# barathanaslan/whisper-ipa

Measured on AMD Instinct MI355X. Metric: audio-seconds/sec transcribed (whisper-small, 30s clips), higher is better.
Workload: dtype bf16

## Files before the change

include/wipa.h:

```cpp
#ifndef WIPA_H
#define WIPA_H
#include <stddef.h>
#include <stdint.h>
#ifdef __cplusplus
extern "C" {
#endif

typedef void* wipa_stream_t;

enum { WIPA_F32 = 0, WIPA_BF16 = 1, WIPA_FP8_E4M3 = 2  };
enum { WIPA_OK = 0, WIPA_ERR_ARG = -1, WIPA_ERR_HIP = -2, WIPA_ERR_STATE = -3 };

#define WIPA_N_SAMPLES 480000
#define WIPA_N_FRAMES 3000
#define WIPA_N_FFT 400
#define WIPA_HOP 160
#define WIPA_HEAD_DIM 64

int wipa_version(void);
const char* wipa_last_error(void);

int wipa_stream_create(wipa_stream_t* out);
int wipa_stream_create_cu_limited(int n_cus, wipa_stream_t* out);
int wipa_stream_destroy(wipa_stream_t s);
// ... 137 lines not shown
    const float* slabs;
    const float* bias_o;
    const float* ln_w;
    const float* ln_b;
    const void* wq;
    const float* bq;
    const void* kv;
    void* out;
    int64_t slab_stride;
    int32_t n_slabs, B, d, H, Tk, dtype;
    float eps, qk_scale;
    int32_t cross_splits;
} wipa_cross_block_desc;
int wipa_decode_cross_block(const wipa_cross_block_desc* d, wipa_stream_t s);

int wipa_cross_absorbed_splits(int want, int Tk);
int wipa_cross_absorbed_resident_groups_for(int B, int d, int Tk, int n_splits, int64_t budget_bytes);
int wipa_cross_absorbed_resident_groups(int B, int d, int Tk, int n_splits);
size_t wipa_cross_absorbed_scratch_bytes(int B, int d, int Tk);
int wipa_cross_absorbed_init(int d);
int wipa_cross_absorbed_attention(const void* q, int64_t q_row_stride, const void* wkT, const void* xa, const void* wv, const float* bv,
                                  void* out, int64_t out_row_stride, void* scratch, size_t scratch_bytes, int B, int H, int d, int Tk,
                                  float k_scale, int n_splits, wipa_stream_t s);
int wipa_decode_cross_absorbed_block(const wipa_cross_block_desc* c, const void* wkT, const void* wv, const float* bv, void* scratch,
                                     size_t scratch_bytes, wipa_stream_t s);
int wipa_decode_cross_absorbed_block_out(const wipa_cross_block_desc* c, const void* wkT, const void* wv, const float* bv, const void* wo,
                                         const float* bo, float* slabs_out, int64_t slab_stride, void* scratch, size_t scratch_bytes,
                                         wipa_stream_t s);
int wipa_cross_absorbed_stream(const void* xa, void* scratch, size_t scratch_bytes, int B, int H, int d, int Tk, int n_splits,
                               wipa_stream_t s);

int wipa_greedy_step(const float* logits, int64_t ldl, int B, int V, const float* mask_first,
                     const float* mask_always, int32_t* tokens, int64_t ld_tok, const int32_t* pos_dev, int n_init,
                     int eot, float* sum_logprobs, int32_t* not_done, wipa_stream_t s);
int wipa_add_i32(int32_t* p, int32_t v, wipa_stream_t s);
int wipa_greedy_step_embed(const float* logits, int64_t ldl, int B, int V, const float* mask_first, const float* mask_always,
                           int32_t* tokens, int64_t ld_tok, int32_t* pos_dev, int64_t* posd_dev, int32_t* done_counter, int n_init,
                           int eot, float* sum_logprobs, int32_t* not_done, const void* tok_emb, int emb_dtype,
                           const float* emb_scale, const float* pos_emb, int n_ctx, float* x, const float* ln_w, const float* ln_b,
                           void* y, int y_dtype, int D, float eps, wipa_stream_t s);
#define WIPA_GREEDY_PARTS 2048
int wipa_logits_greedy_supported(int B, int V, int d, int dtype);
size_t wipa_logits_greedy_partials_bytes(int B);
int wipa_logits_greedy(const void* x, int64_t ldx, const void* w, int64_t ldw, float* logits, int64_t ldl, int B, int V, int d,
                       const float* mask_first, const float* mask_always, const int32_t* pos_dev, int n_init, float* partials,
                       size_t partials_bytes, wipa_stream_t s);
// ... 196 lines not shown
```

whisper_ipa_amd/_lib.py:

```python
from __future__ import annotations

import ctypes as C
import os
import threading

_HERE = os.path.dirname(os.path.abspath(__file__))
LIB_PATH = os.path.join(_HERE, "libwipa.so")

WIPA_F32, WIPA_BF16, WIPA_FP8_E4M3 = 0, 1, 2
GREEDY_PARTS = 2048
RESAMPLE_TILE = 512
SCORE_MAX_LEN = 1024
ENC_GLOBAL, ENC_PER_LAYER = 7, 14
DEC_GLOBAL, DEC_PER_LAYER, DEC_FP8_PER_LAYER = 4, 20, 6
GEMM_DISPATCH = ("tile128", "tile256", "tile384", "tile384n", "tile256p", "skinny", "skinny_fp8", "skinny_ln", "kmajor", "split_k",
                 "tile_fp8", "tile_fp8_384")
ENC_FP8_PER_LAYER = 8
DEC_ABSORBED_PER_LAYER = 1

c_void_p, c_int, c_int64, c_size_t, c_float = C.c_void_p, C.c_int, C.c_int64, C.c_size_t, C.c_float


class GemmDesc(C.Structure):
    _fields_ = [
# ... 88 lines not shown
                               c_float, c_void_p]),
    "wipa_layernorm_fp8": (c_int, [c_void_p, c_int64, c_void_p, c_int64, c_void_p, c_void_p, c_void_p, c_int, c_int, c_float, c_void_p]),
    "wipa_rowquant_fp8": (c_int, [c_void_p, c_int, c_int64, c_void_p, c_int64, c_void_p, c_int, c_int, c_void_p]),
    "wipa_add_slabs_layernorm": (c_int, [c_void_p, c_int64, c_void_p, c_int, c_int64, c_void_p, c_int, c_int64, c_void_p,
                                         c_void_p, c_int, c_int, c_float, c_void_p]),
    "wipa_embed_tokens": (c_int, [c_void_p, c_int64, c_int, c_int, c_int, c_void_p, c_void_p, c_int, c_void_p, c_void_p, c_void_p,
                                  c_int, c_void_p]),
    "wipa_attention": (c_int, [_P(AttnDesc), c_void_p]),
    "wipa_flash_attn_enc_f32": (c_int, [c_void_p, c_int64, c_void_p, c_int64, c_void_p, c_int64, c_void_p, c_int64, c_int, c_int,
                                       c_int, c_int, c_void_p]),
    "wipa_flash_attn_enc_bf16": (c_int, [c_void_p, c_int64, c_void_p, c_int64, c_void_p, c_int64, c_int, c_int, c_int,
                                         c_void_p]),
    "wipa_decode_attn": (c_int, [_P(AttnDesc), c_void_p]),
    "wipa_decode_cross_attn": (c_int, [c_void_p, c_void_p, c_void_p, c_int, c_int, c_int, c_int, c_void_p]),
    "wipa_decode_self_block": (c_int, [_P(SelfBlockDesc), c_void_p]),
    "wipa_decode_cross_block": (c_int, [_P(CrossBlockDesc), c_void_p]),
    "wipa_cross_absorbed_splits": (c_int, [c_int, c_int]),
    "wipa_cross_absorbed_resident_groups_for": (c_int, [c_int, c_int, c_int, c_int, c_int64]),
    "wipa_cross_absorbed_resident_groups": (c_int, [c_int, c_int, c_int, c_int]),
    "wipa_cross_absorbed_scratch_bytes": (c_size_t, [c_int, c_int, c_int]),
    "wipa_cross_absorbed_init": (c_int, [c_int]),
    "wipa_cross_absorbed_attention": (c_int, [c_void_p, c_int64, c_void_p, c_void_p, c_void_p, c_void_p, c_void_p, c_int64, c_void_p, c_size_t,
                                              c_int, c_int, c_int, c_int, c_float, c_int, c_void_p]),
    "wipa_cross_absorbed_stream": (c_int, [c_void_p, c_void_p, c_size_t, c_int, c_int, c_int, c_int, c_int, c_void_p]),
    "wipa_decode_cross_absorbed_block": (c_int, [_P(CrossBlockDesc), c_void_p, c_void_p, c_void_p, c_void_p, c_size_t, c_void_p]),
    "wipa_decode_cross_absorbed_block_out": (c_int, [_P(CrossBlockDesc), c_void_p, c_void_p, c_void_p, c_void_p, c_void_p, c_void_p, c_int64,
                                                     c_void_p, c_size_t, c_void_p]),
    "wipa_greedy_step": (c_int, [c_void_p, c_int64, c_int, c_int, c_void_p, c_void_p, c_void_p, c_int64, c_void_p, c_int,
                                 c_int, c_void_p, c_void_p, c_void_p]),
    "wipa_add_i32": (c_int, [c_void_p, C.c_int32, c_void_p]),
    "wipa_greedy_step_embed": (c_int, [c_void_p, c_int64, c_int, c_int, c_void_p, c_void_p, c_void_p, c_int64, c_void_p, c_void_p, c_void_p,
                                       c_int, c_int, c_void_p, c_void_p, c_void_p, c_int, c_void_p, c_void_p, c_int, c_void_p, c_void_p,
                                       c_void_p, c_void_p, c_int, c_int, c_float, c_void_p]),
    "wipa_timestamp_step": (c_int, [c_void_p, c_int64, c_int, c_int, c_void_p, c_void_p, c_void_p, c_int64, c_void_p, c_int, c_int,
                                    _P(DecodeRules), c_void_p, c_void_p, c_void_p]),
    "wipa_timestamp_step_embed": (c_int, [c_void_p, c_int64, c_int, c_int, c_void_p, c_void_p, c_void_p, c_int64, c_void_p, c_void_p, c_void_p,
                                          c_int, c_int, _P(DecodeRules), c_void_p, c_void_p, c_void_p, c_int, c_void_p, c_void_p, c_int,
                                          c_void_p, c_void_p, c_void_p, c_void_p, c_int, c_int, c_float, c_void_p]),
    "wipa_sample_record_bytes": (c_size_t, [c_int]),
    "wipa_sample_record_fill": (c_int, [c_void_p, c_size_t, C.c_uint64, c_int, c_float, c_void_p, c_int]),
    "wipa_sample_step": (c_int, [c_void_p, c_int64, c_int, c_int, c_void_p, c_void_p, c_void_p, c_int64, c_void_p, c_int, c_int,
                                 _P(DecodeRules), c_void_p, c_void_p, c_void_p, c_void_p]),
    "wipa_sample_step_embed": (c_int, [c_void_p, c_int64, c_int, c_int, c_void_p, c_void_p, c_void_p, c_int64, c_void_p, c_void_p, c_void_p,
                                       c_int, c_int, _P(DecodeRules), c_void_p, c_void_p, c_void_p, c_void_p, c_int, c_void_p, c_void_p, c_int,
                                       c_void_p, c_void_p, c_void_p, c_void_p, c_int, c_int, c_float, c_void_p]),
    "wipa_sample_noise": (c_int, [c_void_p, c_int, c_int, c_int, c_void_p, c_void_p]),
# ... 118 lines not shown
```

whisper_ipa_amd/csrc/cross_absorbed.hip:

```cpp
#include <cstdlib>
#include <mutex>
#include <type_traits>

#include "attn_stream.h"
#include "wipa_common.h"

int wipa_cross_absorbed_loop_variant() {
    const char* e = getenv("WIPA_ABS_LOOP");
    const int v = e ? atoi(e) : 1;
    return (v >= 0 && v <= 3) ? v : 1;
}

namespace {

constexpr int FT = 32;
constexpr long long XA_RESIDENT_MB_SHARED = 16;
constexpr long long XA_RESIDENT_MB_LONE = -1;
typedef __attribute__((address_space(3))) void* lds_ptr_a;
typedef int v2i32 __attribute__((ext_vector_type(2)));

struct AbsParams {
    const __bf16* qp;
    const __bf16* xa;
    float* part_m;
    float* part_l;
    float* part_o;
    int Tk, n_splits, tiles_per_split, H;
    int resident_groups;
};

constexpr int POLICY_DEFAULT = 0, POLICY_NT = 2;

__device__ __forceinline__ int swz(int row) { return (row & 7) << 1; }

template <int D>
struct AbsCfg {
    static constexpr int NW = 4;
    static constexpr int ROWB = D * 2;
    static constexpr int TILE = FT * ROWB;
    static constexpr int SX = NW * 2 * 64 * 4 * (int)sizeof(float);
    static constexpr int NBUF = (3 * TILE + SX <= 160 * 1024) ? 3 : 2;
    static constexpr int SMEM = NBUF * TILE + SX;
};

template <int D>
__global__ __launch_bounds__(512, 1) void cross_absorbed_kernel(AbsParams p) {
    typedef AbsCfg<D> X;
    constexpr int NW = X::NW, ROWB = X::ROWB, TILE = X::TILE, NBUF = X::NBUF;
    constexpr int NDMA = TILE / 1024 / NW;
    constexpr int KS = D / NW / 32;
    constexpr int CT = D / NW / 16;
// ... 242 lines not shown
    return fmaxf(__uint_as_float(r[0]), __uint_as_float(r[1]));
}
__device__ __forceinline__ float sum_xor16(float v) {
    const auto r = __builtin_amdgcn_permlane16_swap(__float_as_uint(v), __float_as_uint(v), false, false);
    return __uint_as_float(r[0]) + __uint_as_float(r[1]);
}
__device__ __forceinline__ float sum_xor32(float v) {
    const auto r = __builtin_amdgcn_permlane32_swap(__float_as_uint(v), __float_as_uint(v), false, false);
    return __uint_as_float(r[0]) + __uint_as_float(r[1]);
}

template <int D, int NW_, bool PIPE>
__global__ __launch_bounds__(64 * NW_, 1) void cross_absorbed_v2_kernel(AbsParams p) {
    typedef AbsCfg2<D, NW_> X;
    constexpr int NWV = X::NWV, GF = X::GF, ROWB = X::ROWB, SLOT = X::SLOT;
    constexpr int NDMA = SLOT / 1024;
    constexpr int KS = D / 32;
    constexpr int CT = D / 16;
    static_assert(SLOT % 1024 == 0 && NDMA <= 32 && CT % 8 == 0 && KS % 4 == 0 && CT / 8 <= 8 && D % 128 == 0, "width");
    extern __shared__ __attribute__((aligned(1024))) char smem[];
    const int tid = threadIdx.x, lane = tid & 63;
    const int wave = __builtin_amdgcn_readfirstlane(tid >> 6);
    const int l15 = lane & 15, g = lane >> 4;
    const int split = blockIdx.x, b = blockIdx.y;
    const int groups_total = (p.Tk + GF - 1) / GF;
    const int gps = 2 * p.tiles_per_split;
    const int g0 = split * gps;
    const int ng = max(0, min(gps, groups_total - g0));
    const int my_n = ng > wave ? (ng - wave + NWV - 1) / NWV : 0;
    const __bf16* xb = p.xa + (int64_t)b * p.Tk * D;
    char* my = smem + wave * (2 * SLOT);

    bf16x8 qf[KS];
    {
        const __bf16* qr = p.qp + ((int64_t)b * 16 + l15) * D + 8 * g;
#pragma unroll
        for (int ks = 0; ks < KS; ++ks) qf[ks] = *reinterpret_cast<const bf16x8*>(qr + 32 * ks);
    }
    const __amdgpu_buffer_rsrc_t rX = __builtin_amdgcn_make_buffer_rsrc((void*)xb, 0, 0x7fffffff, 0x00020000);
    constexpr int G1K = (ROWB % 1024 == 0) ? 1024 : ((ROWB % 512 == 0) ? 512 : 256);
    constexpr int PER = ROWB / G1K, QR = 1024 / G1K;
    static_assert(NDMA % PER == 0 && PER <= 3 && (QR == 1 || QR == 2 || QR == 4), "transfer / row period");
    int dma_a[PER], dma_b[PER];
#pragma unroll
    for (int t = 0; t < PER; ++t) {
        const int off = 1024 * t + 16 * lane;
        const int r = off / ROWB, c = (off - r * ROWB) >> 4;
        dma_a[t] = (c ^ (r << 1)) << 4;
        dma_b[t] = r * ROWB;
    }
    int lane_v = lane;
    auto stage_as = [&](auto policy, int i_local, int slot) {
        constexpr int AUX = decltype(policy)::value;
        const int f0 = (g0 + wave + NWV * i_local) * GF;
        if (f0 + GF <= p.Tk) {
#pragma unroll
            for (int i = 0; i < NDMA; ++i) {
                const int j = i / PER, t = i % PER;
// ... 166 lines not shown
            (void)scores(slot, i, mx);
            mt = fmaxf(mt, mx);
            asm volatile("s_waitcnt lgkmcnt(0)" ::: "memory");
            if (i + 2 < my_n) stage(i + 2, slot);
        }
        m_ref = mt;
        exact = true;
    }
    const float m_run = m_ref;
    asm volatile("s_waitcnt vmcnt(0)" ::: "memory");
    __syncthreads();
    constexpr int RS = X::MROW;
    float* so = reinterpret_cast<float*>(smem);
    float* sm = so + NWV * 16 * RS;
#pragma unroll
    for (int c = 0; c < CT; ++c)
#pragma unroll
        for (int r = 0; r < 4; ++r) so[(wave * 16 + 4 * g + r) * RS + 16 * c + l15] = acc[c][r];
    if (g == 0) {
        sm[wave * 16 + l15] = m_run;
        sm[NWV * 16 + wave * 16 + l15] = l_run;
    }
    __syncthreads();
    const int64_t ps = (int64_t)b * p.n_splits + split;
    float* po = p.part_o + ps * 16 * D;
    for (int hd = 0; hd < p.H; ++hd) {
        float mv[NWV], M = NEG_BIG;
#pragma unroll
        for (int v = 0; v < NWV; ++v) {
            mv[v] = sm[v * 16 + hd];
            M = fmaxf(M, mv[v]);
        }
        float wgt[NWV];
#pragma unroll
        for (int v = 0; v < NWV; ++v) wgt[v] = __expf(mv[v] - M);
        for (int c4 = tid; 4 * c4 < D; c4 += NWV * 64) {
            f32x4 o = {0.f, 0.f, 0.f, 0.f};
#pragma unroll
            for (int v = 0; v < NWV; ++v)
                o += wgt[v] * *reinterpret_cast<const f32x4*>(so + (v * 16 + hd) * RS + 4 * c4);
            *reinterpret_cast<f32x4*>(po + hd * D + 4 * c4) = o;
        }
    }
    if (tid < 16) {
        float M = NEG_BIG, Lsum = 0.f;
#pragma unroll
        for (int v = 0; v < NWV; ++v) M = fmaxf(M, sm[v * 16 + tid]);
#pragma unroll
        for (int v = 0; v < NWV; ++v) Lsum += __expf(sm[v * 16 + tid] - M) * sm[NWV * 16 + v * 16 + tid];
        p.part_m[ps * 16 + tid] = M;
        p.part_l[ps * 16 + tid] = Lsum;
    }
}
#undef WIPA_TR8
#undef WIPA_TR8_ISSUE
#undef WIPA_TR8_NEXT
#undef WIPA_TR8_LAST

template <int D>
__global__ __launch_bounds__(64) void cross_absorb_q_kernel(const __bf16* __restrict__ q, int64_t q_rs, const __bf16* __restrict__ wkT,
                                                            __bf16* __restrict__ qp, int B, int H, float scale) {
    constexpr int CT = D / 4 / 16;
    const int lane = threadIdx.x & 63, wave = blockIdx.z;
    const int l15 = lane & 15, g = lane >> 4;
    const int h = blockIdx.x, b0 = blockIdx.y * 16;
    if (h >= H) {
        for (int e = lane; e < 16 * (D / 4); e += 64) {
            const int bb = b0 + e / (D / 4);
            if (bb < B) qp[((int64_t)bb * 16 + h) * D + wave * (D / 4) + e % (D / 4)] = (__bf16)0.f;
        }
        return;
    }
    const int bq = min(b0 + l15, B - 1);
    bf16x8 qa[2];
#pragma unroll
    for (int ks = 0; ks < 2; ++ks) qa[ks] = *reinterpret_cast<const bf16x8*>(q + (int64_t)bq * q_rs + h * 64 + 32 * ks + 8 * g);
    bf16x8 wb[CT][2];
#pragma unroll
    for (int i = 0; i < CT; ++i)
#pragma unroll
        for (int ks = 0; ks < 2; ++ks)
            wb[i][ks] = *reinterpret_cast<const bf16x8*>(wkT + (int64_t)(wave * (D / 4) + 16 * i + l15) * D + h * 64 + 32 * ks + 8 * g);
#pragma unroll
    for (int i = 0; i < CT; ++i) {
        const int c0 = wave * (D / 4) + 16 * i;
        f32x4 acc = f32x4{0.f, 0.f, 0.f, 0.f};
// ... 6 lines not shown
        }
    }
}

template <int D>
struct MergeCfg {
#ifndef WIPA_MERGE_KQ
#define WIPA_MERGE_KQ 96
#endif
#ifndef WIPA_MERGE_CL
#define WIPA_MERGE_CL 4
#endif
    static constexpr int KQ = (D % 96 == 0) ? WIPA_MERGE_KQ : (D == 512 ? 64 : 128);
    static constexpr int NWM = D / KQ;
    static constexpr int KS = KQ / 32;
    static constexpr int CL = WIPA_MERGE_CL;
};

template <int D, bool OUTP = false, int NS = 4>
__global__ __launch_bounds__(64 * MergeCfg<D>::NWM) void cross_merge_proj_kernel(
    const float* __restrict__ part_m, const float* __restrict__ part_l, const float* __restrict__ part_o, int n_splits,
    const __bf16* __restrict__ wv, const float* __restrict__ bv, __bf16* __restrict__ out, int64_t o_rs, int B,
    const __bf16* __restrict__ wo = nullptr, const float* __restrict__ bo = nullptr, float* __restrict__ slabs_out = nullptr,
    int64_t slab_stride = 0) {
    constexpr int KQ = MergeCfg<D>::KQ, KS = MergeCfg<D>::KS, NWM = MergeCfg<D>::NWM;
    static_assert(KQ % 32 == 0 && NWM * KQ == D, "width");
    constexpr int CL = MergeCfg<D>::CL;
    constexpr int NTO = D / 16;
    constexpr int NTOW = (NTO + NWM - 1) / NWM;
    __shared__ __attribute__((aligned(16))) float red[NWM][CL][64 + 4];
    __shared__ __attribute__((aligned(16))) __bf16 vh[OUTP ? CL : 1][64 + 8];
    const int tid = threadIdx.x, lane = tid & 63, w = tid >> 6;
    const int l15 = lane & 15, g = lane >> 4;
    const int h = blockIdx.x, b0 = blockIdx.y * CL;
    const int bc = min(b0 + (l15 & (CL - 1)), B - 1);
    bf16x8 wq[4][KS];
#pragma unroll
    for (int nt = 0; nt < 4; ++nt)
#pragma unroll
        for (int ks = 0; ks < KS; ++ks)
            wq[nt][ks] = *reinterpret_cast<const bf16x8*>(wv + (int64_t)(h * 64 + 16 * nt + l15) * D + w * KQ + 32 * ks + 8 * g);
    bf16x8 wof[OUTP ? NTOW : 1][2];
    if constexpr (OUTP) {
#pragma unroll
        for (int i = 0; i < NTOW; ++i) {
            const int nt = min(w * NTOW + i, NTO - 1);
#pragma unroll
            for (int ks = 0; ks < 2; ++ks)
// ... 241 lines not shown
                    if (4 * g + r < CG && bb_ < p.B) p.qp[((int64_t)bb_ * 16 + h) * D + 16 * nt + l15] = (__bf16)(acc[r] * p.k_scale);
                }
            }
        }
    }
}

template <int D, bool OUTP, typename... Args>
void launch_merge(int lv, int S, dim3 grid, hipStream_t s, Args... args) {
    constexpr int T = 64 * MergeCfg<D>::NWM;
    const int ns = (lv == 1 || lv == 3) ? S : 4;
    if (ns == 1) hipLaunchKernelGGL((cross_merge_proj_kernel<D, OUTP, 1>), grid, dim3(T), 0, s, args...);
    else if (ns == 2) hipLaunchKernelGGL((cross_merge_proj_kernel<D, OUTP, 2>), grid, dim3(T), 0, s, args...);
    else if (ns == 3) hipLaunchKernelGGL((cross_merge_proj_kernel<D, OUTP, 3>), grid, dim3(T), 0, s, args...);
    else hipLaunchKernelGGL((cross_merge_proj_kernel<D, OUTP, 4>), grid, dim3(T), 0, s, args...);
}

template <int D>
int launch_attn(int lv, const AbsParams& p_in, int B, hipStream_t s) {
    const char* e = getenv("WIPA_ABS_KERNEL");
    const bool pipe = lv == 1 || lv == 2;
    AbsParams p = p_in;
    p.resident_groups = wipa_cross_absorbed_resident_groups(B, D, p.Tk, p.n_splits);
    if ((e && atoi(e) == 1) || (D > 768 && !(e && atoi(e) == 2)))
        hipLaunchKernelGGL((cross_absorbed_kernel<D>), dim3(p.n_splits, B), dim3(64 * AbsCfg<D>::NW), AbsCfg<D>::SMEM, s, p);
    else if constexpr (D > 768) {
        if (pipe) hipLaunchKernelGGL((cross_absorbed_v2_kernel<D, 2, true>), dim3(p.n_splits, B), dim3(128), (AbsCfg2<D, 2>::SMEM), s, p);
        else hipLaunchKernelGGL((cross_absorbed_v2_kernel<D, 2, false>), dim3(p.n_splits, B), dim3(128), (AbsCfg2<D, 2>::SMEM), s, p);
    } else {
        static const int waves = [] { const char* w = getenv("WIPA_ABS_WAVES"); return w ? atoi(w) : 3; }();
        if (waves == 2 && pipe) hipLaunchKernelGGL((cross_absorbed_v2_kernel<D, 2, true>), dim3(p.n_splits, B), dim3(128), (AbsCfg2<D, 2>::SMEM), s, p);
        else if (waves == 2) hipLaunchKernelGGL((cross_absorbed_v2_kernel<D, 2, false>), dim3(p.n_splits, B), dim3(128), (AbsCfg2<D, 2>::SMEM), s, p);
        else if (pipe) hipLaunchKernelGGL((cross_absorbed_v2_kernel<D, 3, true>), dim3(p.n_splits, B), dim3(192), (AbsCfg2<D, 3>::SMEM), s, p);
        else hipLaunchKernelGGL((cross_absorbed_v2_kernel<D, 3, false>), dim3(p.n_splits, B), dim3(192), (AbsCfg2<D, 3>::SMEM), s, p);
    }
    return WIPA_OK;
}

AbsParams abs_params(void* scratch, int B, int d, int Tk, int S, int H, const void* xa) {
    char* sc = (char*)scratch;
    AbsParams p = {};
    p.qp = (const __bf16*)sc; p.xa = (const __bf16*)xa;
    p.part_m = (float*)(sc + (size_t)B * 16 * d * 2);
    p.part_l = p.part_m + (size_t)B * S * 16;
    p.part_o = p.part_l + (size_t)B * S * 16;
    p.Tk = Tk; p.n_splits = S; p.H = H;
    const int tiles = (Tk + FT - 1) / FT;
    p.tiles_per_split = (tiles + S - 1) / S;
    return p;
}

template <typename F>
int for_width(int d, F f) {
    if (d == 384) return f(std::integral_constant<int, 384>());
    if (d == 512) return f(std::integral_constant<int, 512>());
    if (d == 768) return f(std::integral_constant<int, 768>());
    if (d == 1024) return f(std::integral_constant<int, 1024>());
    return WIPA_ERR_ARG;
}

}

extern "C" int wipa_cross_absorbed_splits(int want, int Tk) {
    const int tiles = (Tk + FT - 1) / FT;
    static const int dflt = [] { const char* e = getenv("WIPA_ABS_SPLITS"); const int v = e ? atoi(e) : 4; return (v >= 1 && v <= 4) ? v : 4; }();
    int s = (want >= 1 && want <= 4) ? want : dflt;
    if (s > tiles / 2) s = tiles / 2;
    return s < 1 ? 1 : s;
}

extern "C" int wipa_cross_absorbed_resident_groups_for(int B, int d, int Tk, int n_splits, int64_t budget_bytes) {
    if (B < 1 || d < 1 || Tk < 1) return 0;
    const int S = wipa_cross_absorbed_splits(n_splits, Tk);
    const int tiles = (Tk + FT - 1) / FT;
    const int gps = 2 * ((tiles + S - 1) / S);
    if (budget_bytes < 0 || budget_bytes >= (int64_t)B * Tk * d * 2) return gps;
    const int64_t g = budget_bytes / ((int64_t)B * S * 16 * d * 2);
    return g < gps ? (int)g : gps;
}

extern "C" int wipa_cross_absorbed_resident_groups(int B, int d, int Tk, int n_splits) {
    static const int64_t env_mb = [] { const char* e = getenv("WIPA_XA_RESIDENT_MB"); return e ? (int64_t)atoll(e) : (int64_t)INT64_MIN; }();
    const int S = wipa_cross_absorbed_splits(n_splits, Tk);
    int64_t mb = env_mb;
    if (mb == INT64_MIN) mb = (S <= 2) ? XA_RESIDENT_MB_SHARED : XA_RESIDENT_MB_LONE;
    return wipa_cross_absorbed_resident_groups_for(B, d, Tk, S, mb < 0 ? -1 : mb * 1000000);
}

extern "C" size_t wipa_cross_absorbed_scratch_bytes(int B, int d, int Tk) {
    (void)Tk;
    return (size_t)B * 16 * d * 2 + (size_t)B * 4 * 16 * (2 + (size_t)d) * 4 + 1024;
}

extern "C" int wipa_cross_absorbed_init(int d) {
    static std::mutex mu;
    static bool done[4] = {false, false, false, false};
    const int wi = d == 384 ? 0 : d == 512 ? 1 : d == 768 ? 2 : d == 1024 ? 3 : -1;
    if (wi < 0) return WIPA_ERR_ARG;
    std::lock_guard<std::mutex> lk(mu);
    if (done[wi]) return WIPA_OK;
    hipError_t e = hipSuccess;
    for_width(d, [&](auto width) {
        constexpr int D = decltype(width)::value;
        e = hipFuncSetAttribute(reinterpret_cast<const void*>(&cross_absorbed_kernel<D>), hipFuncAttributeMaxDynamicSharedMemorySize,
                                AbsCfg<D>::SMEM);
        if constexpr (D <= 768) {
            if (e == hipSuccess)
                e = hipFuncSetAttribute(reinterpret_cast<const void*>(&cross_absorbed_v2_kernel<D, 3, true>),
                                        hipFuncAttributeMaxDynamicSharedMemorySize, AbsCfg2<D, 3>::SMEM);
            if (e == hipSuccess)
                e = hipFuncSetAttribute(reinterpret_cast<const void*>(&cross_absorbed_v2_kernel<D, 3, false>),
                                        hipFuncAttributeMaxDynamicSharedMemorySize, AbsCfg2<D, 3>::SMEM);
        }
        if (e == hipSuccess)
// ... 33 lines not shown
    WIPA_REQUIRE(B > 0 && B <= 65535 && H >= 1 && H <= 16 && d == H * 64 && (d == 384 || d == 512 || d == 768 || d == 1024) && Tk >= 1,
                 "wipa_cross_absorbed_attention: bf16, <= 16 heads of 64, d in {384, 512, 768, 1024} (got H=%d d=%d)", H, d);
    WIPA_REQUIRE(q_row_stride % 8 == 0 && out_row_stride >= d && ((uintptr_t)q % 16) == 0 && ((uintptr_t)xa % 16) == 0 &&
                     ((uintptr_t)wkT % 16) == 0 && ((uintptr_t)wv % 16) == 0 && ((uintptr_t)scratch % 16) == 0,
                 "wipa_cross_absorbed_attention: operands must be 16-byte aligned");
    WIPA_REQUIRE((int64_t)Tk * d * 2 < ((int64_t)1 << 31), "wipa_cross_absorbed_attention: clip too long for 32-bit tile offsets");
    WIPA_REQUIRE(scratch_bytes >= wipa_cross_absorbed_scratch_bytes(B, d, Tk), "wipa_cross_absorbed_attention: scratch too small");
    hipStream_t s = (hipStream_t)stream;
    {
        const int rc0 = wipa_cross_absorbed_init(d);
        if (rc0 != WIPA_OK) return rc0;
    }
    const int S = wipa_cross_absorbed_splits(n_splits, Tk);
    const AbsParams p = abs_params(scratch, B, d, Tk, S, H, xa);
    const dim3 gq(16, (B + 15) / 16, 4), gm(H, (B + WIPA_MERGE_CL - 1) / WIPA_MERGE_CL);
    const int lv = wipa_cross_absorbed_loop_variant();
    const char* st_env = getenv("WIPA_ABS_STAGES");
    const int stages = st_env ? atoi(st_env) : 7;
    const int rc = for_width(d, [&](auto width) {
        constexpr int D = decltype(width)::value;
        int rc = WIPA_OK;
        if (stages & 1)
            hipLaunchKernelGGL((cross_absorb_q_kernel<D>), gq, dim3(64), 0, s, (const __bf16*)q, q_row_stride, (const __bf16*)wkT,
                               const_cast<__bf16*>(p.qp), B, H, k_scale);
        if (stages & 2) rc = launch_attn<D>(lv, p, B, s);
        if (rc == WIPA_OK && (stages & 4))
            launch_merge<D, false>(lv, S, gm, s, (const float*)p.part_m, (const float*)p.part_l, (const float*)p.part_o, S, (const __bf16*)wv, bv,
                                   (__bf16*)out, out_row_stride, B, (const __bf16*)nullptr, (const float*)nullptr, (float*)nullptr, (int64_t)0);
        return rc;
    });
    if (rc != WIPA_OK) return rc;
    WIPA_LAUNCH_CHECK();
    return WIPA_OK;
}

static int absorbed_block(const wipa_cross_block_desc* c, const void* wkT, const void* wv, const float* bv, const void* wo, const float* bo,
                          float* slabs_out, int64_t slab_stride, void* scratch, size_t scratch_bytes, wipa_stream_t stream);

extern "C" int wipa_decode_cross_absorbed_block(const wipa_cross_block_desc* c, const void* wkT, const void* wv, const float* bv, void* scratch,
                                                size_t scratch_bytes, wipa_stream_t stream) {
    WIPA_REQUIRE(c && c->out, "wipa_decode_cross_absorbed_block: null pointer");
    return absorbed_block(c, wkT, wv, bv, nullptr, nullptr, nullptr, 0, scratch, scratch_bytes, stream);
}

extern "C" int wipa_decode_cross_absorbed_block_out(const wipa_cross_block_desc* c, const void* wkT, const void* wv, const float* bv,
                                                    const void* wo, const float* bo, float* slabs_out, int64_t slab_stride, void* scratch,
                                                    size_t scratch_bytes, wipa_stream_t stream) {
    WIPA_REQUIRE(c && wo && bo && slabs_out && slab_stride >= (int64_t)c->B * c->d && ((uintptr_t)wo % 16) == 0,
                 "wipa_decode_cross_absorbed_block_out: null pointer / short slab stride");
    return absorbed_block(c, wkT, wv, bv, wo, bo, slabs_out, slab_stride, scratch, scratch_bytes, stream);
}
// ... 10 lines not shown
                 "wipa_decode_cross_absorbed_block: bf16, <= 16 heads of 64, d in {384, 512, 768, 1024}, <= 4 slabs, no separate bias, "
                 "cross_splits 0..4");
    WIPA_REQUIRE(c->n_slabs == 0 || c->slabs, "wipa_decode_cross_absorbed_block: slabs missing");
    WIPA_REQUIRE((int64_t)Tk * d * 2 < ((int64_t)1 << 31), "wipa_decode_cross_absorbed_block: clip too long for 32-bit tile offsets");
    WIPA_REQUIRE(scratch_bytes >= wipa_cross_absorbed_scratch_bytes(B, d, Tk), "wipa_decode_cross_absorbed_block: scratch too small");
    hipStream_t s = (hipStream_t)stream;
    const int S = wipa_cross_absorbed_splits(c->cross_splits, Tk);
    const AbsParams p = abs_params(scratch, B, d, Tk, S, H, c->kv);
    AbsPrologueParams q = {};
    q.x_in = c->x_in; q.x_out = c->x_out; q.slabs = c->slabs; q.ln_w = c->ln_w; q.ln_b = c->ln_b;
    q.wq = (const __bf16*)c->wq; q.bq = c->bq; q.wkT = (const __bf16*)wkT; q.qp = const_cast<__bf16*>(p.qp);
    q.slab_stride = c->slab_stride; q.n_slabs = c->n_slabs; q.B = B; q.H = H;
    q.eps = c->eps; q.q_scale = c->qk_scale; q.k_scale = c->qk_scale;
    const int lv = wipa_cross_absorbed_loop_variant();
    static const int cg = [] { const char* e = getenv("WIPA_ABS_PROLOGUE_CLIPS"); return e ? atoi(e) : 8; }();
    const dim3 gp(H, cg == 8 ? (B + 7) / 8 : (B + 15) / 16), gm(H, (B + WIPA_MERGE_CL - 1) / WIPA_MERGE_CL);
    const int rc = for_width(d, [&](auto width) {
        constexpr int D = decltype(width)::value;
        if (cg == 8) hipLaunchKernelGGL((cross_absorb_prologue_kernel<D, 8>), gp, dim3(512), 0, s, q);
        else hipLaunchKernelGGL((cross_absorb_prologue_kernel<D, 16>), gp, dim3(512), 0, s, q);
        const int rc = launch_attn<D>(lv, p, B, s);
        if (rc == WIPA_OK && wo)
            launch_merge<D, true>(lv, S, gm, s, (const float*)p.part_m, (const float*)p.part_l, (const float*)p.part_o, S, (const __bf16*)wv, bv,
                                  (__bf16*)nullptr, (int64_t)d, B, (const __bf16*)wo, bo, slabs_out, slab_stride);
        else if (rc == WIPA_OK)
            launch_merge<D, false>(lv, S, gm, s, (const float*)p.part_m, (const float*)p.part_l, (const float*)p.part_o, S, (const __bf16*)wv, bv,
                                   (__bf16*)c->out, (int64_t)d, B, (const __bf16*)nullptr, (const float*)nullptr, (float*)nullptr, (int64_t)0);
        return rc;
    });
    if (rc != WIPA_OK) return rc;
    WIPA_LAUNCH_CHECK();
    return WIPA_OK;
}
```

whisper_ipa_amd/csrc/runtime.hip:

```cpp
#include <algorithm>
#include <cstdarg>
#include <cstdlib>
#include <cstring>
#include <strings.h>
#include <map>
#include <mutex>
#include <tuple>
#include <vector>

#include "wipa_common.h"

static thread_local char g_err[512] = "";
void wipa_set_error(const char* fmt, ...) {
    va_list ap;
    va_start(ap, fmt);
    vsnprintf(g_err, sizeof(g_err), fmt, ap);
    va_end(ap);
}
extern "C" const char* wipa_last_error(void) { return g_err; }
extern "C" int wipa_version(void) { return 100; }

extern "C" int wipa_stream_create_cu_limited(int n_cus, wipa_stream_t* out) {
    int dev = 0, total = 0;
    WIPA_CHECK_HIP(hipGetDevice(&dev));
// ... 264 lines not shown
    size_t x, x2, ln, q, ao, h, slabs, posd, absorbed, greedy_part, total;
};
inline int k_slices_for(int K, int dtype) {
    const int ksteps = K * (int)wipa_dtype_size(dtype) / 64;
    int s = ksteps / 12;
    return s < 1 ? 1 : (s > MAX_SLABS ? MAX_SLABS : s);
}
int decode_mode(const wipa_model_cfg* cfg, int B);
constexpr int MAX_PROMPT = 4;
DecScratch dec_scratch(const wipa_model_cfg* c, int B) {
    const size_t e = wipa_dtype_size(c->dtype), d = c->n_text_state;
    const size_t R = (size_t)B * MAX_PROMPT;
    DecScratch s;
    size_t o = 0;
    s.x = o;    o += align256(R * d * 4);
    s.x2 = o;   o += align256((size_t)B * d * 4);
    s.ln = o;   o += align256(R * d * e);
    s.q = o;    o += align256(R * d * e);
    s.ao = o;   o += align256(R * d * e);
    s.h = o;    o += align256(R * 4 * d * e);
    s.slabs = o; o += align256(std::max((size_t)MAX_SLABS * R, (size_t)c->n_text_head * B) * d * 4);
    s.posd = o; o += 256;
    s.absorbed = o;
    if (c->dec_cross_absorbed) o += align256(wipa_cross_absorbed_scratch_bytes(B, (int)d, c->n_audio_ctx));
    s.greedy_part = o;
    if (wipa_logits_greedy_supported(B, c->n_vocab, (int)d, c->dtype)) o += align256(wipa_logits_greedy_partials_bytes(B));
    s.total = o;
    return s;
}

wipa_dec_layout dec_layout(const wipa_model_cfg* c, int B) {
    const size_t e = wipa_dtype_size(c->dtype);
    const size_t d = c->n_text_state, H = c->n_text_head;
    wipa_dec_layout L;
    size_t o = 0;
    L.ld_tok = c->n_text_ctx + 8;
    L.tokens = o; o += align256((size_t)B * L.ld_tok * 4);
    L.pos = o; o += 256;
    L.not_done = o; o += 256;
    L.sum_logprobs = o; o += align256((size_t)B * 4);
    L.ld_logits = round_up(c->n_vocab, 8);
    L.logits = o; o += align256((size_t)B * L.ld_logits * 4);
    L.cross_kv = o; o += align256(c->dec_cross_absorbed ? (size_t)B * c->n_audio_ctx * d * e
                                                        : (size_t)c->n_text_layer * B * 2 * H * c->n_audio_ctx * 64 * e);
    L.self_kv = o; o += align256((size_t)c->n_text_layer * 3 * B * c->n_text_ctx * d * e);
    L.scratch = o; o += dec_scratch(c, B).total;
    L.total_bytes = o;
// ... 1 lines not shown
}

__global__ void advance_pos_kernel(int32_t* pos, int64_t* posd, int d) {
    const int p = *pos + 1;
    *pos = p;
    *posd = (int64_t)p * d;
}

__global__ void fill_tokens_kernel(int32_t* tokens, int64_t ld_tok, int B, int n_init, int i0, int i1, int i2, int i3) {
    const int b = blockIdx.x * blockDim.x + threadIdx.x;
    if (b >= B) return;
    const int first4[4] = {i0, i1, i2, i3};
    for (int t = 0; t < n_init; ++t) tokens[(int64_t)b * ld_tok + t] = first4[t & 3];
}

bool absorbed_block_fused() {
    const char* e = getenv("WIPA_ABS_FUSED_PROLOGUE");
    return !(e && atoi(e) == 0);
}

bool absorbed_merge_out() {
    const char* e = getenv("WIPA_ABS_MERGE_OUT");
    return e && atoi(e) == 1;
}
bool tail_fused() {
    const char* e = getenv("WIPA_DECODE_TAIL");
    return !(e && atoi(e) == 0);
}
thread_local bool t_lean_logits = false;
thread_local const wipa_decode_rules* t_rules = nullptr;
thread_local const void* t_sample = nullptr;
thread_local const int32_t* t_starts = nullptr;
bool logits_fused(const wipa_model_cfg* cfg, int B) {
    const char* e = getenv("WIPA_LOGITS_FUSED");
    const bool on = !(e && atoi(e) == 0);
    return on && !t_rules && !t_sample && !t_starts && tail_fused() && cfg->dec_w_dtype == 0 && wipa_logits_greedy_supported(B, cfg->n_vocab, cfg->n_text_state, cfg->dtype);
}
int32_t* done_counter_of(char* st, const wipa_dec_layout& L) { return (int32_t*)(st + L.pos + 64); }

int enqueue_step_head(const wipa_model_cfg* cfg, const void* const* w, char* st, const wipa_dec_layout& L, int B, wipa_stream_t stream) {
    const DecScratch S = dec_scratch(cfg, B);
    char* sc = st + L.scratch;
    const void* const* lw0 = w + WIPA_DEC_GLOBAL;
    if (t_starts)
        return wipa_embed_layernorm_ragged((const int32_t*)(st + L.tokens), L.ld_tok, B, (const int32_t*)(st + L.pos), t_starts, w[0], emb_dtype(cfg),
                                           emb_scale(cfg, w), (const float*)w[1], cfg->n_text_ctx, (float*)(sc + S.x), (const float*)lw0[0],
// ... 289 lines not shown
            RT_CALL(gemm(ln, d, lw[2], d, skv, d, M, 3 * d, d, dt, dt, (const float*)lw[3], 0, nullptr, stream, &g));
        }
        {
            wipa_attn_desc a;
            memset(&a, 0, sizeof(a));
            const size_t slot = (size_t)B * nctx * d * e;
            a.q = skv; a.k = skv + slot; a.v = skv + 2 * slot; a.out = ao;
            a.q_bs = (int64_t)nctx * d; a.q_rs = d; a.q_hs = 64;
            a.k_bs = a.q_bs; a.k_rs = d; a.k_hs = 64;
            a.v_bs = a.q_bs; a.v_rs = d; a.v_hs = 64;
            a.o_bs = (int64_t)P * d; a.o_rs = d; a.o_hs = 64;
            a.B = B; a.H = H; a.Tq = P; a.Tk = P; a.causal = 1; a.dtype = dt;
            RT_CALL(wipa_attention(&a, stream));
        }
        RT_CALL(residual_gemm(ao, d, lw[4], lw[5]));
        RT_CALL(ln_step(lw[6], lw[7]));
        {
            wipa_gemm_desc g;
            memset(&g, 0, sizeof(g));
        g.stream_weights = 1;
            g.col_scale_n = d; g.col_scale = QK_SCALE;
            RT_CALL(gemm(ln, d, lw[8], d, q, d, M, d, d, dt, dt, (const float*)lw[9], 0, nullptr, stream, &g));
        }
        if (cfg->dec_cross_absorbed) {
            const void* wkT = w[WIPA_DEC_GLOBAL + WIPA_DEC_PER_LAYER * cfg->n_text_layer + WIPA_DEC_ABSORBED_PER_LAYER * l];
            for (int t = 0; t < P; ++t)
                RT_CALL(wipa_cross_absorbed_attention((const char*)q + (size_t)t * d * e, (int64_t)P * d, wkT, st + L.cross_kv,
                                                      (const char*)lw[10] + (size_t)d * d * e, (const float*)lw[11] + d,
                                                      (char*)ao + (size_t)t * d * e, (int64_t)P * d, sc + S.absorbed, S.greedy_part - S.absorbed, B,
                                                      H, d, Ta, QK_SCALE, cfg->dec_cross_splits, stream));
        } else {
            RT_CALL(wipa_decode_cross_attn_multi(q, ckv, ao, B, H, Ta, P, dt, stream));
        }
        RT_CALL(residual_gemm(ao, d, lw[12], lw[13]));
        RT_CALL(ln_step(lw[14], lw[15]));
        {
            wipa_gemm_desc g;
            memset(&g, 0, sizeof(g));
            g.stream_weights = 1;
            RT_CALL(gemm(ln, d, lw[16], d, hb, 4 * d, M, 4 * d, d, dt, dt, (const float*)lw[17], 1, nullptr, stream, &g));
        }
        RT_CALL(residual_gemm(hb, 4 * d, lw[18], lw[19]));
    }
    RT_CALL(ln_step(w[2], w[3]));
    float* logits = (float*)(st + L.logits);
    RT_CALL(gemm(ln + (size_t)(P - 1) * d * e, (int64_t)P * d, w[0], d, logits, L.ld_logits, B, cfg->n_vocab, d, dt, WIPA_F32, nullptr, 0,
                 nullptr, stream));
// ... 328 lines not shown
    RT_CALL(cfg_check(cfg));
    SplitScope split_scope(cfg);
    WIPA_REQUIRE(w && state && mask_first && mask_always && B > 0, "wipa_decoder_prefill: bad arguments");
    RT_CALL(rules_servable("wipa_decoder_prefill_rules", cfg, B, eot, rules));
    RT_CALL(sample_servable("wipa_decoder_prefill_sample", cfg, B, sample));
    RulesScope rules_scope(rules, sample);
    WIPA_REQUIRE(n_init >= 1 && n_init <= MAX_PROMPT, "wipa_decoder_prefill: 1..%d prompt tokens (got %d)", MAX_PROMPT, n_init);
    W8Scope w8_scope(cfg, w);
    const wipa_dec_layout L = dec_layout(cfg, B);
    RT_CALL(state_fits("wipa_decoder_prefill", L, state_bytes));
    char* st = (char*)state;
    auto enqueue = [&]() -> int {
        if (n_init == 1) {
            if (step_needs_head(cfg, B)) RT_CALL(enqueue_step_head(cfg, w, st, L, B, stream));
            return enqueue_decode_step(cfg, w, st, L, B, n_init, eot, mask_first, mask_always, stream);
        }
        return enqueue_prefill(cfg, w, st, L, B, n_init, eot, mask_first, mask_always, stream);
    };
    hipStream_t s = (hipStream_t)stream;
    RT_CALL(init_before_capture(cfg));
    WIPA_CHECK_HIP(hipMemsetAsync(done_counter_of(st, L), 0, sizeof(int32_t), s));
    if (!use_graph || s == nullptr || !graphs_allowed()) return enqueue();
    hipGraphExec_t exec = nullptr;
    RT_CALL(cached_graph(graph_key(cfg, w, state, mask_first, mask_always, B, n_init, eot, step_variant(cfg, B), 1, rules, sample, nullptr, nullptr), s,
                         enqueue, &exec));
    WIPA_CHECK_HIP(hipGraphLaunch(exec, s));
    return WIPA_OK;
}

namespace {
struct PromptWs {
    size_t sot_logits, x, ln, q, ao, h, ckv, total;
};
PromptWs prompt_ws(const wipa_model_cfg* c, int B, int P) {
    const size_t e = wipa_dtype_size(c->dtype), d = c->n_text_state, M = (size_t)B * P;
    PromptWs w;
    size_t o = 0;
    w.sot_logits = o; o += align256((size_t)B * round_up(c->n_vocab, 8) * 4);
    w.x = o;   o += align256(M * d * 4);
    w.ln = o;  o += align256(M * d * e);
    w.q = o;   o += align256(M * d * e);
    w.ao = o;  o += align256(M * d * e);
    w.h = o;   o += align256(M * 4 * d * e);
    w.ckv = o; o += c->dec_cross_absorbed ? align256((size_t)B * 2 * c->n_text_head * c->n_audio_ctx * 64 * e) : 0;
    w.total = o;
    return w;
}

// ... 377 lines not shown
```

Baseline: 27050.

## Batch all prompt rows into one absorbed cross-attention launch during prefill

Prefill previously ran the absorbed cross-attention once per prompt token, issuing three kernels per row per layer. A new rows entry point folds the prompt rows into the grid (z dimension for q-absorb and merge, an interleaved chunk index for the attention kernel), so each layer launches three kernels total. Rows that share an encoder-KV tile are scheduled next to each other for cache reuse. Scratch space grows to hold partials for MAX_PROMPT rows, and the path is on by default through an environment switch.

```diff
diff --git a/include/wipa.h b/include/wipa.h
--- a/include/wipa.h
+++ b/include/wipa.h
@@ -183,6 +183,10 @@
 int wipa_cross_absorbed_attention(const void* q, int64_t q_row_stride, const void* wkT, const void* xa, const void* wv, const float* bv,
                                   void* out, int64_t out_row_stride, void* scratch, size_t scratch_bytes, int B, int H, int d, int Tk,
                                   float k_scale, int n_splits, wipa_stream_t s);
+size_t wipa_cross_absorbed_scratch_bytes_rows(int B, int d, int Tk, int P);
+int wipa_cross_absorbed_attention_rows(const void* q, int64_t q_row_stride, const void* wkT, const void* xa, const void* wv, const float* bv,
+                                       void* out, int64_t out_row_stride, void* scratch, size_t scratch_bytes, int B, int P, int H, int d,
+                                       int Tk, float k_scale, int n_splits, wipa_stream_t s);
 int wipa_decode_cross_absorbed_block(const wipa_cross_block_desc* c, const void* wkT, const void* wv, const float* bv, void* scratch,
                                      size_t scratch_bytes, wipa_stream_t s);
 int wipa_decode_cross_absorbed_block_out(const wipa_cross_block_desc* c, const void* wkT, const void* wv, const float* bv, const void* wo,
diff --git a/whisper_ipa_amd/_lib.py b/whisper_ipa_amd/_lib.py
--- a/whisper_ipa_amd/_lib.py
+++ b/whisper_ipa_amd/_lib.py
@@ -134,6 +134,9 @@
     "wipa_cross_absorbed_init": (c_int, [c_int]),
     "wipa_cross_absorbed_attention": (c_int, [c_void_p, c_int64, c_void_p, c_void_p, c_void_p, c_void_p, c_void_p, c_int64, c_void_p, c_size_t,
                                               c_int, c_int, c_int, c_int, c_float, c_int, c_void_p]),
+    "wipa_cross_absorbed_scratch_bytes_rows": (c_size_t, [c_int, c_int, c_int, c_int]),
+    "wipa_cross_absorbed_attention_rows": (c_int, [c_void_p, c_int64, c_void_p, c_void_p, c_void_p, c_void_p, c_void_p, c_int64, c_void_p,
+                                                   c_size_t, c_int, c_int, c_int, c_int, c_int, c_float, c_int, c_void_p]),
     "wipa_cross_absorbed_stream": (c_int, [c_void_p, c_void_p, c_size_t, c_int, c_int, c_int, c_int, c_int, c_void_p]),
     "wipa_decode_cross_absorbed_block": (c_int, [_P(CrossBlockDesc), c_void_p, c_void_p, c_void_p, c_void_p, c_size_t, c_void_p]),
     "wipa_decode_cross_absorbed_block_out": (c_int, [_P(CrossBlockDesc), c_void_p, c_void_p, c_void_p, c_void_p, c_void_p, c_void_p, c_int64,
diff --git a/whisper_ipa_amd/csrc/cross_absorbed.hip b/whisper_ipa_amd/csrc/cross_absorbed.hip
--- a/whisper_ipa_amd/csrc/cross_absorbed.hip
+++ b/whisper_ipa_amd/csrc/cross_absorbed.hip
@@ -27,6 +27,8 @@
     float* part_o;
     int Tk, n_splits, tiles_per_split, H;
     int resident_groups;
+    int rows;
+    int64_t qp_rs, part_rs;
 };
 
 constexpr int POLICY_DEFAULT = 0, POLICY_NT = 2;
@@ -315,7 +317,22 @@
     const int tid = threadIdx.x, lane = tid & 63;
     const int wave = __builtin_amdgcn_readfirstlane(tid >> 6);
     const int l15 = lane & 15, g = lane >> 4;
-    const int split = blockIdx.x, b = blockIdx.y;
+    int split, b, t = 0;
+    if (p.rows > 1) {
+        const int n_pairs = gridDim.x / p.rows, per = 8 * p.rows;
+        const int chunk = blockIdx.x / per, r = blockIdx.x - chunk * per;
+        const int w = min(8, n_pairs - 8 * chunk);
+        t = r / w;
+        const int pair = 8 * chunk + (r - t * w);
+        b = pair / p.n_splits;
+        split = pair - b * p.n_splits;
+        t = __builtin_amdgcn_readfirstlane(t);
+        b = __builtin_amdgcn_readfirstlane(b);
+        split = __builtin_amdgcn_readfirstlane(split);
+    } else {
+        split = blockIdx.x;
+        b = blockIdx.y;
+    }
     const int groups_total = (p.Tk + GF - 1) / GF;
     const int gps = 2 * p.tiles_per_split;
     const int g0 = split * gps;
@@ -326,7 +343,7 @@
 
     bf16x8 qf[KS];
     {
-        const __bf16* qr = p.qp + ((int64_t)b * 16 + l15) * D + 8 * g;
+        const __bf16* qr = p.qp + (int64_t)t * p.qp_rs + ((int64_t)b * 16 + l15) * D + 8 * g;
 #pragma unroll
         for (int ks = 0; ks < KS; ++ks) qf[ks] = *reinterpret_cast<const bf16x8*>(qr + 32 * ks);
     }
@@ -539,7 +556,7 @@
         sm[NWV * 16 + wave * 16 + l15] = l_run;
     }
     __syncthreads();
-    const int64_t ps = (int64_t)b * p.n_splits + split;
+    const int64_t ps = (int64_t)t * p.part_rs + (int64_t)b * p.n_splits + split;
     float* po = p.part_o + ps * 16 * D;
     for (int hd = 0; hd < p.H; ++hd) {
         float mv[NWV], M = NEG_BIG;
@@ -576,9 +593,11 @@
 
 template <int D>
 __global__ __launch_bounds__(64) void cross_absorb_q_kernel(const __bf16* __restrict__ q, int64_t q_rs, const __bf16* __restrict__ wkT,
-                                                            __bf16* __restrict__ qp, int B, int H, float scale) {
+                                                            __bf16* __restrict__ qp, int B, int H, float scale, int64_t q_ts, int64_t qp_ts) {
     constexpr int CT = D / 4 / 16;
-    const int lane = threadIdx.x & 63, wave = blockIdx.z;
+    const int lane = threadIdx.x & 63, wave = blockIdx.z & 3;
+    q += (int64_t)(blockIdx.z >> 2) * q_ts;
+    qp += (int64_t)(blockIdx.z >> 2) * qp_ts;
     const int l15 = lane & 15, g = lane >> 4;
     const int h = blockIdx.x, b0 = blockIdx.y * 16;
     if (h >= H) {
@@ -631,8 +650,14 @@
     const float* __restrict__ part_m, const float* __restrict__ part_l, const float* __restrict__ part_o, int n_splits,
     const __bf16* __restrict__ wv, const float* __restrict__ bv, __bf16* __restrict__ out, int64_t o_rs, int B,
     const __bf16* __restrict__ wo = nullptr, const float* __restrict__ bo = nullptr, float* __restrict__ slabs_out = nullptr,
-    int64_t slab_stride = 0) {
+    int64_t slab_stride = 0, int64_t part_ts = 0, int64_t out_ts = 0) {
     constexpr int KQ = MergeCfg<D>::KQ, KS = MergeCfg<D>::KS, NWM = MergeCfg<D>::NWM;
+    if constexpr (!OUTP) {
+        part_m += (int64_t)blockIdx.z * part_ts * 16;
+        part_l += (int64_t)blockIdx.z * part_ts * 16;
+        part_o += (int64_t)blockIdx.z * part_ts * 16 * D;
+        out += (int64_t)blockIdx.z * out_ts;
+    }
     static_assert(KQ % 32 == 0 && NWM * KQ == D, "width");
     constexpr int CL = MergeCfg<D>::CL;
     constexpr int NTO = D / 16;
@@ -920,6 +945,16 @@
     const bool pipe = lv == 1 || lv == 2;
     AbsParams p = p_in;
     p.resident_groups = wipa_cross_absorbed_resident_groups(B, D, p.Tk, p.n_splits);
+    if (p.rows > 1) {
+        p.resident_groups = 2 * p.tiles_per_split;
+        const dim3 grid((unsigned)(p.n_splits * B * p.rows));
+        if constexpr (D <= 768) {
+            if (pipe) hipLaunchKernelGGL((cross_absorbed_v2_kernel<D, 3, true>), grid, dim3(192), (AbsCfg2<D, 3>::SMEM), s, p);
+            else hipLaunchKernelGGL((cross_absorbed_v2_kernel<D, 3, false>), grid, dim3(192), (AbsCfg2<D, 3>::SMEM), s, p);
+            return WIPA_OK;
+        }
+        return WIPA_ERR_ARG;
+    }
     if ((e && atoi(e) == 1) || (D > 768 && !(e && atoi(e) == 2)))
         hipLaunchKernelGGL((cross_absorbed_kernel<D>), dim3(p.n_splits, B), dim3(64 * AbsCfg<D>::NW), AbsCfg<D>::SMEM, s, p);
     else if constexpr (D > 768) {
@@ -935,13 +970,20 @@
     return WIPA_OK;
 }
 
-AbsParams abs_params(void* scratch, int B, int d, int Tk, int S, int H, const void* xa) {
+bool rows_kernel_chosen(int d) {
+    const char* e = getenv("WIPA_ABS_KERNEL");
+    const char* w = getenv("WIPA_ABS_WAVES");
+    return d <= 768 && !(e && atoi(e) == 1) && !(w && atoi(w) == 2);
+}
+
+AbsParams abs_params(void* scratch, int B, int d, int Tk, int S, int H, const void* xa, int R = 1) {
     char* sc = (char*)scratch;
     AbsParams p = {};
     p.qp = (const __bf16*)sc; p.xa = (const __bf16*)xa;
-    p.part_m = (float*)(sc + (size_t)B * 16 * d * 2);
-    p.part_l = p.part_m + (size_t)B * S * 16;
-    p.part_o = p.part_l + (size_t)B * S * 16;
+    p.part_m = (float*)(sc + (size_t)R * B * 16 * d * 2);
+    p.part_l = p.part_m + (size_t)R * B * S * 16;
+    p.part_o = p.part_l + (size_t)R * B * S * 16;
+    p.rows = R; p.qp_rs = (int64_t)B * 16 * d; p.part_rs = (int64_t)B * S;
     p.Tk = Tk; p.n_splits = S; p.H = H;
     const int tiles = (Tk + FT - 1) / FT;
     p.tiles_per_split = (tiles + S - 1) / S;
@@ -988,6 +1030,12 @@
 extern "C" size_t wipa_cross_absorbed_scratch_bytes(int B, int d, int Tk) {
     (void)Tk;
     return (size_t)B * 16 * d * 2 + (size_t)B * 4 * 16 * (2 + (size_t)d) * 4 + 1024;
+}
+
+extern "C" size_t wipa_cross_absorbed_scratch_bytes_rows(int B, int d, int Tk, int P) {
+    (void)Tk;
+    if (P < 1) P = 1;
+    return (size_t)P * ((size_t)B * 16 * d * 2 + (size_t)B * 4 * 16 * (2 + (size_t)d) * 4) + 1024;
 }
 
 extern "C" int wipa_cross_absorbed_init(int d) {
@@ -1067,11 +1115,62 @@
         int rc = WIPA_OK;
         if (stages & 1)
             hipLaunchKernelGGL((cross_absorb_q_kernel<D>), gq, dim3(64), 0, s, (const __bf16*)q, q_row_stride, (const __bf16*)wkT,
-                               const_cast<__bf16*>(p.qp), B, H, k_scale);
+                               const_cast<__bf16*>(p.qp), B, H, k_scale, (int64_t)0, (int64_t)0);
         if (stages & 2) rc = launch_attn<D>(lv, p, B, s);
         if (rc == WIPA_OK && (stages & 4))
             launch_merge<D, false>(lv, S, gm, s, (const float*)p.part_m, (const float*)p.part_l, (const float*)p.part_o, S, (const __bf16*)wv, bv,
-                                   (__bf16*)out, out_row_stride, B, (const __bf16*)nullptr, (const float*)nullptr, (float*)nullptr, (int64_t)0);
+                                   (__bf16*)out, out_row_stride, B, (const __bf16*)nullptr, (const float*)nullptr, (float*)nullptr, (int64_t)0,
+                                   (int64_t)0, (int64_t)0);
+        return rc;
+    });
+    if (rc != WIPA_OK) return rc;
+    WIPA_LAUNCH_CHECK();
+    return WIPA_OK;
+}
+
+extern "C" int wipa_cross_absorbed_attention_rows(const void* q, int64_t q_row_stride, const void* wkT, const void* xa, const void* wv,
+                                                  const float* bv, void* out, int64_t out_row_stride, void* scratch, size_t scratch_bytes,
+                                                  int B, int P, int H, int d, int Tk, float k_scale, int n_splits, wipa_stream_t stream) {
+    WIPA_REQUIRE(P >= 1 && P <= 8, "wipa_cross_absorbed_attention_rows: 1..8 query rows per clip (got %d)", P);
+    if (P == 1 || !rows_kernel_chosen(d)) {
+        for (int t = 0; t < P; ++t) {
+            const int rc = wipa_cross_absorbed_attention((const __bf16*)q + (size_t)t * d, q_row_stride, wkT, xa, wv, bv, (__bf16*)out + (size_t)t * d,
+                                                         out_row_stride, scratch, scratch_bytes, B, H, d, Tk, k_scale, n_splits, stream);
+            if (rc != WIPA_OK) return rc;
+        }
+        return WIPA_OK;
+    }
+    WIPA_REQUIRE(q && wkT && xa && wv && bv && out && scratch, "wipa_cross_absorbed_attention_rows: null pointer");
+    WIPA_REQUIRE(n_splits >= 0 && n_splits <= 4, "wipa_cross_absorbed_attention_rows: n_splits %d (0 = default, 1..4)", n_splits);
+    WIPA_REQUIRE(B > 0 && B <= 65535 && H >= 1 && H <= 16 && d == H * 64 && (d == 384 || d == 512 || d == 768) && Tk >= 1,
+                 "wipa_cross_absorbed_attention_rows: bf16, <= 16 heads of 64, d in {384, 512, 768} (got H=%d d=%d)", H, d);
+    WIPA_REQUIRE(q_row_stride % 8 == 0 && q_row_stride >= (int64_t)P * d && out_row_stride >= (int64_t)P * d && ((uintptr_t)q % 16) == 0 &&
+                     ((uintptr_t)xa % 16) == 0 && ((uintptr_t)wkT % 16) == 0 && ((uintptr_t)wv % 16) == 0 && ((uintptr_t)scratch % 16) == 0,
+                 "wipa_cross_absorbed_attention_rows: operands must be 16-byte aligned, row strides >= P * d");
+    WIPA_REQUIRE((int64_t)Tk * d * 2 < ((int64_t)1 << 31), "wipa_cross_absorbed_attention_rows: clip too long for 32-bit tile offsets");
+    WIPA_REQUIRE(scratch_bytes >= wipa_cross_absorbed_scratch_bytes_rows(B, d, Tk, P), "wipa_cross_absorbed_attention_rows: scratch too small");
+    hipStream_t s = (hipStream_t)stream;
+    {
+        const int rc0 = wipa_cross_absorbed_init(d);
+        if (rc0 != WIPA_OK) return rc0;
+    }
+    const int S = wipa_cross_absorbed_splits(n_splits, Tk);
+    const AbsParams p = abs_params(scratch, B, d, Tk, S, H, xa, P);
+    const dim3 gq(16, (B + 15) / 16, 4 * P), gm(H, (B + WIPA_MERGE_CL - 1) / WIPA_MERGE_CL, P);
+    const int lv = wipa_cross_absorbed_loop_variant();
+    const char* st_env = getenv("WIPA_ABS_STAGES");
+    const int stages = st_env ? atoi(st_env) : 7;
+    const int rc = for_width(d, [&](auto width) {
+        constexpr int D = decltype(width)::value;
+        int rc = WIPA_OK;
+        if (stages & 1)
+            hipLaunchKernelGGL((cross_absorb_q_kernel<D>), gq, dim3(64), 0, s, (const __bf16*)q, q_row_stride, (const __bf16*)wkT,
+                               const_cast<__bf16*>(p.qp), B, H, k_scale, (int64_t)d, p.qp_rs);
+        if (stages & 2) rc = launch_attn<D>(lv, p, B, s);
+        if (rc == WIPA_OK && (stages & 4))
+            launch_merge<D, false>(lv, S, gm, s, (const float*)p.part_m, (const float*)p.part_l, (const float*)p.part_o, S, (const __bf16*)wv, bv,
+                                   (__bf16*)out, out_row_stride, B, (const __bf16*)nullptr, (const float*)nullptr, (float*)nullptr, (int64_t)0,
+                                   p.part_rs, (int64_t)d);
         return rc;
     });
     if (rc != WIPA_OK) return rc;
@@ -1128,10 +1227,11 @@
         const int rc = launch_attn<D>(lv, p, B, s);
         if (rc == WIPA_OK && wo)
             launch_merge<D, true>(lv, S, gm, s, (const float*)p.part_m, (const float*)p.part_l, (const float*)p.part_o, S, (const __bf16*)wv, bv,
-                                  (__bf16*)nullptr, (int64_t)d, B, (const __bf16*)wo, bo, slabs_out, slab_stride);
+                                  (__bf16*)nullptr, (int64_t)d, B, (const __bf16*)wo, bo, slabs_out, slab_stride, (int64_t)0, (int64_t)0);
         else if (rc == WIPA_OK)
             launch_merge<D, false>(lv, S, gm, s, (const float*)p.part_m, (const float*)p.part_l, (const float*)p.part_o, S, (const __bf16*)wv, bv,
-                                   (__bf16*)c->out, (int64_t)d, B, (const __bf16*)nullptr, (const float*)nullptr, (float*)nullptr, (int64_t)0);
+                                   (__bf16*)c->out, (int64_t)d, B, (const __bf16*)nullptr, (const float*)nullptr, (float*)nullptr, (int64_t)0,
+                                   (int64_t)0, (int64_t)0);
         return rc;
     });
     if (rc != WIPA_OK) return rc;
diff --git a/whisper_ipa_amd/csrc/runtime.hip b/whisper_ipa_amd/csrc/runtime.hip
--- a/whisper_ipa_amd/csrc/runtime.hip
+++ b/whisper_ipa_amd/csrc/runtime.hip
@@ -310,7 +310,7 @@
     s.slabs = o; o += align256(std::max((size_t)MAX_SLABS * R, (size_t)c->n_text_head * B) * d * 4);
     s.posd = o; o += 256;
     s.absorbed = o;
-    if (c->dec_cross_absorbed) o += align256(wipa_cross_absorbed_scratch_bytes(B, (int)d, c->n_audio_ctx));
+    if (c->dec_cross_absorbed) o += align256(wipa_cross_absorbed_scratch_bytes_rows(B, (int)d, c->n_audio_ctx, MAX_PROMPT));
     s.greedy_part = o;
     if (wipa_logits_greedy_supported(B, c->n_vocab, (int)d, c->dtype)) o += align256(wipa_logits_greedy_partials_bytes(B));
     s.total = o;
@@ -358,6 +358,10 @@
 bool absorbed_merge_out() {
     const char* e = getenv("WIPA_ABS_MERGE_OUT");
     return e && atoi(e) == 1;
+}
+bool absorbed_prefill_rows() {
+    const char* e = getenv("WIPA_ABS_PREFILL_ROWS");
+    return !(e && atoi(e) == 0);
 }
 bool tail_fused() {
     const char* e = getenv("WIPA_DECODE_TAIL");
@@ -693,7 +697,12 @@
             g.col_scale_n = d; g.col_scale = QK_SCALE;
             RT_CALL(gemm(ln, d, lw[8], d, q, d, M, d, d, dt, dt, (const float*)lw[9], 0, nullptr, stream, &g));
         }
-        if (cfg->dec_cross_absorbed) {
+        if (cfg->dec_cross_absorbed && absorbed_prefill_rows()) {
+            const void* wkT = w[WIPA_DEC_GLOBAL + WIPA_DEC_PER_LAYER * cfg->n_text_layer + WIPA_DEC_ABSORBED_PER_LAYER * l];
+            RT_CALL(wipa_cross_absorbed_attention_rows(q, (int64_t)P * d, wkT, st + L.cross_kv, (const char*)lw[10] + (size_t)d * d * e,
+                                                       (const float*)lw[11] + d, ao, (int64_t)P * d, sc + S.absorbed, S.greedy_part - S.absorbed,
+                                                       B, P, H, d, Ta, QK_SCALE, cfg->dec_cross_splits, stream));
+        } else if (cfg->dec_cross_absorbed) {
             const void* wkT = w[WIPA_DEC_GLOBAL + WIPA_DEC_PER_LAYER * cfg->n_text_layer + WIPA_DEC_ABSORBED_PER_LAYER * l];
             for (int t = 0; t < P; ++t)
                 RT_CALL(wipa_cross_absorbed_attention((const char*)q + (size_t)t * d * e, (int64_t)P * d, wkT, st + L.cross_kv,
@@ -1068,8 +1077,10 @@
     WIPA_CHECK_HIP(hipMemsetAsync(done_counter_of(st, L), 0, sizeof(int32_t), s));
     if (!use_graph || s == nullptr || !graphs_allowed()) return enqueue();
     hipGraphExec_t exec = nullptr;
-    RT_CALL(cached_graph(graph_key(cfg, w, state, mask_first, mask_always, B, n_init, eot, step_variant(cfg, B), 1, rules, sample, nullptr, nullptr), s,
-                         enqueue, &exec));
+    RT_CALL(cached_graph(graph_key(cfg, w, state, mask_first, mask_always, B, n_init, eot,
+                                   step_variant(cfg, B) + 65536 * (int)(cfg->dec_cross_absorbed && absorbed_prefill_rows()), 1, rules, sample,
+                                   nullptr, nullptr),
+                         s, enqueue, &exec));
     WIPA_CHECK_HIP(hipGraphLaunch(exec, s));
     return WIPA_OK;
 }
```

Measured after the change: 27120, median of 6. About the same (+0.3%).
